# The-Learning-And-Vision-Atelier-LAVA/BUFFER

Measured on AMD Instinct MI355X. Metric: registration pairs/sec, higher is better.
Workload: dtype f32

## Files before the change

### buffer_amd/csrc/convnet_wg.hip

```cpp
#include "common.h"
#include <type_traits>

#define WG_CS 160
#define WG_ROW 22
#define WG_ZERO 154
#define WG_MAXC 128
#define WG_LAYERS 8
#define WG_THREADS 256
#define WG_BUF (WG_MAXC * WG_CS)
#define WG_KSTEP (16 * WG_CS)
#ifndef WG_PIN_FOLD
#define WG_PIN_FOLD 1
#endif
#define WG_BLOCKS 16
#ifdef WG_EXP_NOBAR
#define WG_SYNC() __builtin_amdgcn_sched_barrier(0)
#else
#define WG_SYNC() __syncthreads()
#endif

typedef float wgf4 __attribute__((ext_vector_type(4)));
typedef float wgf2 __attribute__((ext_vector_type(2)));
typedef const __attribute__((address_space(3))) wgf2* wg_lds_f2;

struct CylWgParams {
    const float* wt[WG_LAYERS];
    const float* bias[WG_LAYERS];
    int cin[WG_LAYERS], cout[WG_LAYERS], relu[WG_LAYERS];
    const int* only_if;
#ifdef WG_STAMP
    long long* stamps;
#endif
};
#ifdef WG_STAMP
__device__ long long* wg_stamp_ptr;
#define WG_STAMP_IN(SLOT) if ((threadIdx.x & 63) == 0) wg_stamp_ptr[((size_t)blockIdx.x * 4 + threadIdx.x / 64) * 20 + (SLOT)] = __builtin_amdgcn_s_memtime();
#define WG_STAMP_AT(SLOT) if ((threadIdx.x & 63) == 0) P.stamps[((size_t)blockIdx.x * 4 + w) * 20 + (SLOT)] = __builtin_amdgcn_s_memtime();
#else
#define WG_STAMP_AT(SLOT)
#define WG_STAMP_IN(SLOT)
#endif

__device__ __forceinline__ bool wg_tile(int t, int idx, int& ty, int& tx)
{
    if (t == 0) { const bool a = idx < 10; ty = a ? 0 : 1; tx = a ? idx : idx - 6; return true; }
    if (t == 1) { const bool a = idx < 10, b = idx < 14; ty = a ? 2 : (b ? 1 : 3); tx = a ? idx : (b ? idx - 10 : idx - 6); return true; }
    ty = 3; tx = idx & 7;
    return idx < 8;
}

__device__ __forceinline__ unsigned wg_row_addr(unsigned act_addr, int t, int a, int li, int lk)
{
    int ty, tx;
    const bool ok = wg_tile(t, li, ty, tx);
    const int row = 2 * ty - 1 + a;
    return act_addr + 4u * (unsigned)(lk * WG_CS + ((ok && row >= 0 && row <= 6) ? row * WG_ROW + 2 * tx : WG_ZERO));
}

__device__ __forceinline__ float wg_add(float a, float b) { float r; asm("v_add_f32 %0, %1, %2" : "=v"(r) : "v"(a), "v"(b)); return r; }
__device__ __forceinline__ float wg_sub(float a, float b) { float r; asm("v_sub_f32 %0, %1, %2" : "=v"(r) : "v"(a), "v"(b)); return r; }

__host__ __device__ constexpr int wg_a1(int I) { return I == 0 ? 0 : 1; }
__host__ __device__ constexpr int wg_a2(int I) { return I == 3 ? 3 : 2; }
__host__ __device__ constexpr int wg_te(int I, int T1) { return (I == 3 && T1 == 3) ? 2 : T1; }

__host__ __device__ constexpr bool wg_chains(int I, int T0, int T1)
{
    if (I < 0 || I >= 3) return false;
    const int nt = wg_te(I, T1) - T0, ntn = wg_te(I + 1, T1) - T0;
    return nt >= 1 && ntn >= 1 && (1 / nt) == (1 / ntn) && (1 % nt) == (1 % ntn);
}

#define WG_LOAD2(DST, A0, A1_, OFS)                                                                       \
    {                                                                                                     \
        DST[0] = *(wg_lds_f2)(size_t)((A0) + (OFS));                                                      \
        asm volatile("" : "+v"(A0));                                                                      \
        DST[1] = *(wg_lds_f2)(size_t)((A0) + (OFS) + 8);                                                  \
        asm volatile("" : "+v"(A0));                                                                      \
        DST[2] = *(wg_lds_f2)(size_t)((A1_) + (OFS));                                                     \
        asm volatile("" : "+v"(A1_));                                                                     \
        DST[3] = *(wg_lds_f2)(size_t)((A1_) + (OFS) + 8);                                                 \
        asm volatile("" : "+v"(A1_));                                                                     \
    }

#define WG_LOAD1(DST, A0, OFS)                                                                            \
    {                                                                                                     \
        DST[0] = *(wg_lds_f2)(size_t)((A0) + (OFS));                                                      \
        asm volatile("" : "+v"(A0));                                                                      \
        DST[1] = *(wg_lds_f2)(size_t)((A0) + (OFS) + 8);                                                  \
        asm volatile("" : "+v"(A0));                                                                      \
    }
#define WG_LOAD(BOT_, DST, A0, A1_, OFS)                                                                  \
    {                                                                                                     \
        if constexpr (BOT_) WG_LOAD1(DST, A0, OFS) else WG_LOAD2(DST, A0, A1_, OFS)                       \
    }

typedef unsigned wgu4 __attribute__((ext_vector_type(4)));
__device__ __forceinline__ __amdgpu_buffer_rsrc_t wg_weights(const float* wt)
{
    return __builtin_amdgcn_make_buffer_rsrc((void*)wt, 0, 0x7fffffff, 0x00027000);
}
__device__ __forceinline__ wgf4 wg_ldw(__amdgpu_buffer_rsrc_t rs, unsigned uniform_float_ofs, unsigned lane_byte_ofs)
{
    return __builtin_bit_cast(wgf4, __builtin_amdgcn_raw_buffer_load_b128(rs, lane_byte_ofs, uniform_float_ofs * 4, 0));
}

template <int I, int NN, int T0, int T1, bool PRIMED, int INEXT, bool BOT = false, unsigned KSTEP = WG_KSTEP, bool DIFF = false>
__device__ __forceinline__ void wg_pass(unsigned (&RA)[3][4], __amdgpu_buffer_rsrc_t rs, unsigned wp, unsigned wp_next, unsigned lofs, int niter,
                                        int wstride, wgf4 (&W)[NN][2], wgf4 (&acc)[NN][3][4], wgf2 (&D)[2][4], wgf4 (*Wb)[2] = nullptr, unsigned bofs = 0)
{
    constexpr int A1 = BOT ? I : wg_a1(I), A2 = BOT ? I : wg_a2(I);
    constexpr int TE = BOT ? T1 : wg_te(I, T1);
    constexpr int NT = TE > T0 ? TE - T0 : 1;
    if constexpr (TE <= T0) return;
    constexpr int A1N = BOT ? (INEXT < 0 ? 0 : INEXT) : wg_a1(INEXT < 0 ? 0 : INEXT), A2N = BOT ? A1N : wg_a2(INEXT < 0 ? 0 : INEXT);
    constexpr int NTN = (INEXT < 0 || BOT) ? NT : (wg_te(INEXT, T1) - T0);
    static_assert(INEXT < 0 || (NTN >= 1 && (1 / NT) == (1 / NTN) && (1 % NT) == (1 % NTN)), "steps 0 and 1 of the chained pass have this pass's shape");
    float V[2][4];
    unsigned P[NT][2];
#pragma unroll
    for (int t = 0; t < NT; t++) { P[t][0] = RA[T0 + t][A1]; P[t][1] = RA[T0 + t][A2]; }
    if constexpr (!PRIMED) {
#pragma unroll
        for (int g = 0; g < 2; g++) WG_LOAD(BOT, D[g], P[g % NT][0], P[g % NT][1], (g / NT) * KSTEP)
    }
#define WG_XFORM(BUF)                                                                                     \
    {                                                                                                     \
        float r_[4];                                                                                      \
        _Pragma("unroll") for (int b = 0; b < 4; b++) {                                                   \
            const float da_ = D[BUF][b >> 1][b & 1];                                                      \
            if constexpr (BOT) r_[b] = da_;                                                               \
            else {                                                                                        \
                const float db_ = D[BUF][2 + (b >> 1)][b & 1];                                            \
                r_[b] = I == 1 ? wg_add(da_, db_) : (I == 2 ? wg_sub(db_, da_) : wg_sub(da_, db_));       \
            }                                                                                             \
        }                                                                                                 \
        V[BUF][0] = wg_sub(r_[0], r_[2]); V[BUF][1] = wg_add(r_[1], r_[2]);                               \
        V[BUF][2] = wg_sub(r_[2], r_[1]); V[BUF][3] = wg_sub(r_[1], r_[3]);                               \
    }
    WG_XFORM(0)
#pragma unroll 1
    for (int it = 0; it < niter; it++) {
        const bool more = it + 1 < niter;
        const unsigned wcur = wp + 4 * it * wstride;
        const unsigned wn = more ? wcur + 4 * wstride : wp_next;
        const unsigned adv = more ? 4u * KSTEP : 0u;
        __builtin_amdgcn_sched_barrier(0);
#pragma unroll
        for (int s = 0; s < 4 * NT; s++) {
            const int t = T0 + s % NT, kk = s / NT, g = s + 2;
            if (g < 4 * NT) WG_LOAD(BOT, D[s & 1], P[g % NT][0], P[g % NT][1], (g / NT) * KSTEP)
            else {
                const int t2 = (g - 4 * NT) % NT;
                if ((g - 4 * NT) / NT == 0) { P[t2][0] += adv; P[t2][1] += adv; }
                if constexpr (INEXT >= 0) {
                    unsigned q0 = more ? P[t2][0] : RA[T0 + t2][A1N], q1 = more ? P[t2][1] : RA[T0 + t2][A2N];
                    WG_LOAD(BOT, D[s & 1], q0, q1, ((g - 4 * NT) / NT) * KSTEP)
                } else
                    WG_LOAD(BOT, D[s & 1], P[t2][0], P[t2][1], ((g - 4 * NT) / NT) * KSTEP)
            }
            __builtin_amdgcn_sched_barrier(0);
            if constexpr (DIFF) {
                wgf4 wd[NN];
#pragma unroll
                for (int n = 0; n < NN; n++)
#pragma unroll
                    for (int j = 0; j < 4; j++) wd[n][j] = wg_sub(W[n][kk & 1][j], Wb[n][kk & 1][j]);
                __builtin_amdgcn_sched_barrier(0);
#pragma unroll
                for (int n = 0; n < NN; n++)
#pragma unroll
                    for (int j = 0; j < 4; j++)
                        acc[n][t][j] = __builtin_amdgcn_mfma_f32_16x16x4f32(wd[n][j], V[s & 1][j], acc[n][t][j], 0, 0, 0);
            } else {
#pragma unroll
                for (int n = 0; n < NN; n++)
#pragma unroll
                    for (int j = 0; j < 4; j++)
                        acc[n][t][j] = __builtin_amdgcn_mfma_f32_16x16x4f32(W[n][kk & 1][j], V[s & 1][j], acc[n][t][j], 0, 0, 0);
            }
            __builtin_amdgcn_sched_barrier(0);
            WG_XFORM((s + 1) & 1)
            if (s % NT == NT - 1) {
#pragma unroll
                for (int n = 0; n < NN; n++)
                    W[n][kk & 1] = kk < 2 ? wg_ldw(rs, wcur + n * 256 + (kk + 2) * wstride, lofs) : wg_ldw(rs, wn + n * 256 + (kk - 2) * wstride, lofs);
                if constexpr (DIFF) {
#pragma unroll
                    for (int n = 0; n < NN; n++)
                        Wb[n][kk & 1] = kk < 2 ? wg_ldw(rs, wcur + bofs + n * 256 + (kk + 2) * wstride, lofs) : wg_ldw(rs, wn + bofs + n * 256 + (kk - 2) * wstride, lofs);
                }
            }
            __builtin_amdgcn_sched_barrier(0);
        }
#pragma unroll
        for (int t = 2; t < NT; t++) { P[t][0] += adv; P[t][1] += adv; }
    }
#undef WG_XFORM
}

template <int NN, int T0, int T1, unsigned KSTEP = WG_KSTEP, bool FENCE = false>
__device__ __forceinline__ void wg_round(unsigned (&RA)[3][4], __amdgpu_buffer_rsrc_t rs, unsigned wp, unsigned wp_after, unsigned lofs, int niter,
                                         int wstride, unsigned pstride, const float* __restrict__ bias_lane, wgf4 (&W)[NN][2], wgf4 (&Y)[NN][3][2][2])
{
    using std::integral_constant;
    wgf2 D[2][4];
    wgf4 bv[NN];
#pragma unroll
    for (int n = 0; n < NN; n++) bv[n] = bias_lane ? *reinterpret_cast<const wgf4*>(bias_lane + n * 16) : (wgf4){ 0.f, 0.f, 0.f, 0.f };
    wgf4 acc[NN][3][4];
    float zero = 0.f;
    asm volatile("" : "+v"(zero));
#pragma unroll
    for (int n = 0; n < NN; n++)
#pragma unroll
        for (int t = T0; t < T1; t++)
#pragma unroll
            for (int j = 0; j < 4; j++) acc[n][t][j] = (wgf4){ zero, zero, zero, zero };
    auto run = [&](auto ic) __attribute__((always_inline)) {
        constexpr int I = decltype(ic)::value;
        constexpr int INEXT = (I == 3 || (I == 2 && wg_te(3, T1) <= T0)) ? 0 : I + 1;
        if constexpr (I == 1) {
#pragma unroll
            for (int n = 0; n < NN; n++)
#pragma unroll
                for (int t = T0; t < T1; t++) acc[n][t][1] += bv[n];
        }
        constexpr int ICHAIN = (INEXT != 0 && wg_chains(I, T0, T1)) ? INEXT : -1;
        wg_pass<I, NN, T0, T1, wg_chains(I - 1, T0, T1), ICHAIN, false, KSTEP>(RA, rs, wp + I * pstride, INEXT == 0 ? wp_after : wp + (I + 1) * pstride, lofs, niter, wstride, W, acc, D);
        if constexpr (FENCE) __builtin_amdgcn_sched_barrier(0);
#pragma unroll
        for (int n = 0; n < NN; n++)
#pragma unroll
            for (int t = T0; t < T1; t++) {
                if (I == 3 && t == 2) continue;
                if (I == 2 ? false : t == 2) continue;
                const wgf4 f0 = acc[n][t][0] + acc[n][t][1] + acc[n][t][2];
                const wgf4 f1 = acc[n][t][1] - acc[n][t][2] - acc[n][t][3];
                if constexpr (I == 0) { Y[n][t][1][0] = f0; Y[n][t][1][1] = f1; }
                else if constexpr (I == 1) {
#pragma unroll
                    for (int r = 0; r < 4; r++) {
                        Y[n][t][1][0][r] = __builtin_fmaf(2.f, f0[r], -Y[n][t][1][0][r]);
                        Y[n][t][1][1][r] = __builtin_fmaf(2.f, f1[r], -Y[n][t][1][1][r]);
                    }
                }
                else if constexpr (I == 2) { Y[n][t][0][0] = f0; Y[n][t][0][1] = f1; }
                else { Y[n][t][1][0] -= f0; Y[n][t][1][1] -= f1; }
                if constexpr (FENCE || WG_PIN_FOLD) {
                    if constexpr (I == 2) asm volatile("" : "+v"(Y[n][t][0][0]), "+v"(Y[n][t][0][1]));
                    else asm volatile("" : "+v"(Y[n][t][1][0]), "+v"(Y[n][t][1][1]));
                }
            }
    };
    run(integral_constant<int, 0>{});
    run(integral_constant<int, 1>{});
    run(integral_constant<int, 2>{});
    run(integral_constant<int, 3>{});
}

template <int NN>
__device__ __forceinline__ void wg_round_bottom(unsigned (&RA)[3][4], __amdgpu_buffer_rsrc_t rs, unsigned wp, unsigned wp_after, unsigned lofs, int niter,
                                                int wstride, unsigned pstride, const float* __restrict__ bias_lane, wgf4 (&W)[NN][2], wgf4 (&Y)[NN][3][2][2])
{
    wgf2 D[2][4];
    wgf4 acc[NN][3][4];
    float zero = 0.f;
    asm volatile("" : "+v"(zero));
#pragma unroll
    for (int n = 0; n < NN; n++)
#pragma unroll
        for (int j = 0; j < 4; j++)
            acc[n][2][j] = (j == 1 && bias_lane) ? *reinterpret_cast<const wgf4*>(bias_lane + n * 16) : (wgf4){ zero, zero, zero, zero };
    wgf4 Wb[NN][2];
#pragma unroll
    for (int n = 0; n < NN; n++)
#pragma unroll
        for (int k = 0; k < 2; k++) Wb[n][k] = wg_ldw(rs, wp + 2 * pstride + n * 256 + k * wstride, lofs);
    wg_pass<0, NN, 2, 3, false, 1, true>(RA, rs, wp, wp + pstride, lofs, niter, wstride, W, acc, D);
    wg_pass<1, NN, 2, 3, true, -1, true, WG_KSTEP, true>(RA, rs, wp + pstride, wp_after, lofs, niter, wstride, W, acc, D, Wb, pstride);
#pragma unroll
    for (int n = 0; n < NN; n++) {
        Y[n][2][0][0] = acc[n][2][0] + acc[n][2][1] + acc[n][2][2];
        Y[n][2][0][1] = acc[n][2][1] - acc[n][2][2] - acc[n][2][3];
    }
}

template <bool GLB, int NU = 2>
__device__ __forceinline__ void wg_store_tile(const wgf4 (&Yt)[2][2], int t, int nt, int relu, float* __restrict__ act, float* __restrict__ out_glb,
                                              int li, int lk)
{
    const int n0 = nt * 16 + lk * 4;
    const float lo = relu ? 0.f : -__builtin_inff();
    {
        int ty, tx;
        const bool valid = wg_tile(t, li, ty, tx);
#pragma unroll
        for (int u = 0; u < NU; u++) {
            const int row = 2 * ty + u;
            const bool ok = valid && row < 7;
            if constexpr (GLB) {
                if (ok) {
#pragma unroll
                    for (int r = 0; r < 4; r++) {
                        const float v0 = fmaxf(Yt[u][0][r], lo), v1 = fmaxf(Yt[u][1][r], lo);
                        *reinterpret_cast<wgf2*>(out_glb + (size_t)(n0 + r) * 140 + row * 20 + 2 * tx) = (wgf2){ v0, v1 };
                    }
                }
            } else {
                const int pos = ok ? row * WG_ROW + 2 * tx + 1 : WG_ZERO + 4;
                const int h0 = (ok && tx == 0) ? row * WG_ROW + 21 : WG_ZERO + 4;
                const int h1 = (ok && tx == 9) ? row * WG_ROW : WG_ZERO + 5;
                float* p = act + n0 * WG_CS;
#pragma unroll
                for (int r = 0; r < 4; r++) {
                    const float v0 = fmaxf(Yt[u][0][r], lo), v1 = fmaxf(Yt[u][1][r], lo);
                    p[r * WG_CS + pos] = v0; p[r * WG_CS + pos + 1] = v1;
                    p[r * WG_CS + h0] = v0; p[r * WG_CS + h1] = v1;
                }
            }
        }
    }
}

template <int T0, int T1, bool GLB>
__device__ __forceinline__ void wg_store(const wgf4 (&Y)[3][2][2], int nt, int relu, float* __restrict__ act, float* __restrict__ out_glb,
                                         int li, int lk)
{
#pragma unroll
    for (int t = T0; t < T1; t++) {
        if (t == 2) wg_store_tile<GLB, 1>(Y[t], t, nt, relu, act, out_glb, li, lk);
        else wg_store_tile<GLB, 2>(Y[t], t, nt, relu, act, out_glb, li, lk);
    }
}

__device__ __forceinline__ void wg_addresses(const float* act, int k0, int li, int lk, unsigned (&RA)[3][4])
{
    const unsigned act_addr = (unsigned)(size_t)(__attribute__((address_space(3))) const float*)act + (unsigned)k0 * WG_KSTEP;
#pragma unroll
    for (int t = 0; t < 3; t++)
#pragma unroll
        for (int a = 0; a < 4; a++) RA[t][a] = wg_row_addr(act_addr, t, a, li, lk);
}

#ifndef WG_ADDR_PARK
#define WG_ADDR_PARK 1
#endif
struct WgAddrPark { float a[3][4]; };
__device__ __forceinline__ void wg_park_addresses(const float* act, int li, int lk, WgAddrPark& pk)
{
    const unsigned act_addr = (unsigned)(size_t)(__attribute__((address_space(3))) const float*)act;
#pragma unroll
    for (int t = 0; t < 3; t++)
#pragma unroll
        for (int a = 0; a < 4; a++) {
            const unsigned v = wg_row_addr(act_addr, t, a, li, lk);
            asm volatile("v_accvgpr_write_b32 %0, %1" : "=a"(pk.a[t][a]) : "v"(v));
        }
}
__device__ __forceinline__ unsigned wg_parked(const WgAddrPark& pk, int t, int a)
{
    unsigned v;
    asm volatile("v_accvgpr_read_b32 %0, %1" : "=v"(v) : "a"(pk.a[t][a]));
    return v;
}

template <int NN, int K0, int K1, int KN>
__device__ __forceinline__ void wg_first_weights(__amdgpu_buffer_rsrc_t rs, unsigned wp, unsigned lofs, int wstride, wgf4 (&W)[NN][KN])
{
#pragma unroll
    for (int n = 0; n < NN; n++)
#pragma unroll
        for (int k = K0; k < K1; k++) W[n][k] = wg_ldw(rs, wp + n * 256 + k * wstride, lofs);
}

#define WG_XCH_C 64
template <bool GLB>
__device__ __forceinline__ void wg_layer_ksplit(float* __restrict__ act, float* __restrict__ out_glb, const float* __restrict__ wt,
                                                const float* __restrict__ bias, int cin, int cout, int relu, int w, const WgAddrPark& pk)
{
    int lane = threadIdx.x & (WAVE - 1);
    asm volatile("" : "+v"(lane));
    const int li = lane & 15, lk = lane >> 4;
    const int nt = w & 1, half = w >> 1;
    const int k4 = cin >> 2, kn = k4 >> 1, k0 = half * kn, wstride = 256;
    unsigned RA[3][4];
#if WG_ADDR_PARK
#pragma unroll
    for (int t = 0; t < 3; t++)
#pragma unroll
        for (int a = 0; a < 4; a++) RA[t][a] = wg_parked(pk, t, a) + (unsigned)k0 * WG_KSTEP;
#else
    wg_addresses(act, k0, li, lk, RA);
#endif
    const __amdgpu_buffer_rsrc_t rs = wg_weights(wt);
    const unsigned wp = (unsigned)nt * (WG_BLOCKS * cin * 16) + (unsigned)k0 * wstride;
    const unsigned lofs = lane * 16;
    wgf4 W[1][2];
    wg_first_weights<1, 0, 2>(rs, wp, lofs, wstride, W);
    wgf4 Y[1][3][2][2];
    wg_round<1, 0, 2>(RA, rs, wp, wp, lofs, kn >> 2, wstride, (unsigned)(k4 * wstride), half ? nullptr : bias + nt * 16 + lk * 4, W, Y);
    wg_round_bottom<1>(RA, rs, wp, wp, lofs, kn >> 2, wstride, (unsigned)(k4 * wstride), half ? nullptr : bias + nt * 16 + lk * 4, W, Y);
    wgf4* slot = reinterpret_cast<wgf4*>(act + WG_XCH_C * WG_CS) + nt * 640 + lane;
    if (half) {
#pragma unroll
        for (int q = 0; q < 10; q++) slot[q * 64] = Y[0][q >> 2][(q >> 1) & 1][q & 1];
    }
    WG_STAMP_IN(18)
    WG_SYNC();
    WG_STAMP_IN(19)
    if (!half) {
#pragma unroll
        for (int q = 0; q < 10; q++) Y[0][q >> 2][(q >> 1) & 1][q & 1] += slot[q * 64];
        wg_store<0, 3, GLB>(Y[0], nt, relu, act, out_glb, li, lk);
    }
}

template <bool GLB>
__device__ __forceinline__ void wg_layer_mksplit(float* __restrict__ act, float* __restrict__ out_glb, const float* __restrict__ wt,
                                                 const float* __restrict__ bias, int cin, int cout, int relu, int w, const WgAddrPark& pk)
{
    int lane = threadIdx.x & (WAVE - 1);
    asm volatile("" : "+v"(lane));
    const int li = lane & 15, lk = lane >> 4;
    const int h = w & 1, half = w >> 1;
    const int k4 = cin >> 2, kn = k4 >> 1, k0 = half * kn, wstride = 512;
    unsigned RA[3][4];
#if WG_ADDR_PARK
#pragma unroll
    for (int a = 0; a < 4; a++) {
        const unsigned r0 = wg_parked(pk, 0, a), r1 = wg_parked(pk, 1, a);
        RA[0][a] = (h ? r1 : r0) + (unsigned)k0 * WG_KSTEP; RA[1][a] = RA[0][a]; RA[2][a] = wg_parked(pk, 2, a) + (unsigned)k0 * WG_KSTEP;
    }
#else
    {
        const unsigned act_addr = (unsigned)(size_t)(__attribute__((address_space(3))) const float*)act + (unsigned)k0 * WG_KSTEP;
#pragma unroll
        for (int a = 0; a < 4; a++) { RA[0][a] = wg_row_addr(act_addr, h, a, li, lk); RA[1][a] = RA[0][a]; RA[2][a] = wg_row_addr(act_addr, 2, a, li, lk); }
    }
#endif
    const __amdgpu_buffer_rsrc_t rs = wg_weights(wt);
    const unsigned wp = (unsigned)k0 * wstride;
    const unsigned wpb = wp + (unsigned)h * 256;
    const unsigned lofs = lane * 16;
    const unsigned pstride = (unsigned)(k4 * wstride);
    wgf4 Y[2][3][2][2];
    wgf4 W2[2][2];
    wg_first_weights<2, 0, 2>(rs, wp, lofs, wstride, W2);
    wg_round<2, 0, 1>(RA, rs, wp, wpb, lofs, kn >> 2, wstride, pstride, half ? nullptr : bias + lk * 4, W2, Y);
    wgf4 W1[1][2] = { { W2[0][0], W2[0][1] } };
    wgf4 Yb[1][3][2][2];
    wg_round_bottom<1>(RA, rs, wpb, wpb, lofs, kn >> 2, wstride, pstride, half ? nullptr : bias + h * 16 + lk * 4, W1, Yb);
    wgf4* slot = reinterpret_cast<wgf4*>(act + WG_XCH_C * WG_CS) + h * 640 + lane;
    if (half) {
#pragma unroll
        for (int q = 0; q < 8; q++) slot[q * 64] = Y[q >> 2][0][(q >> 1) & 1][q & 1];
        slot[8 * 64] = Yb[0][2][0][0]; slot[9 * 64] = Yb[0][2][0][1];
    }
    WG_SYNC();
    if (!half) {
#pragma unroll
        for (int q = 0; q < 8; q++) Y[q >> 2][0][(q >> 1) & 1][q & 1] += slot[q * 64];
        Yb[0][2][0][0] += slot[8 * 64]; Yb[0][2][0][1] += slot[9 * 64];
        wg_store_tile<GLB, 2>(Y[0][0], h, 0, relu, act, out_glb, li, lk);
        wg_store_tile<GLB, 2>(Y[1][0], h, 1, relu, act, out_glb, li, lk);
        wg_store_tile<GLB, 1>(Yb[0][2], 2, h, relu, act, out_glb, li, lk);
    }
}

__device__ __forceinline__ void wg_layer_msplit(float* __restrict__ act, const float* __restrict__ wt, const float* __restrict__ bias,
                                                int cin, int cout, int relu, int w, const WgAddrPark& pk)
{
    int lane = threadIdx.x & (WAVE - 1);
    asm volatile("" : "+v"(lane));
    const int li = lane & 15, lk = lane >> 4;
    const int pair = w & 1, h = w >> 1;
    const int k4 = cin >> 2, wstride = 512;
    unsigned RA[3][4];
#if WG_ADDR_PARK
#pragma unroll
    for (int a = 0; a < 4; a++) {
        const unsigned r0 = wg_parked(pk, 0, a), r1 = wg_parked(pk, 1, a);
        RA[0][a] = h ? r1 : r0; RA[1][a] = RA[0][a]; RA[2][a] = wg_parked(pk, 2, a);
    }
#else
    {
        const unsigned act_addr = (unsigned)(size_t)(__attribute__((address_space(3))) const float*)act;
#pragma unroll
        for (int a = 0; a < 4; a++) { RA[0][a] = wg_row_addr(act_addr, h, a, li, lk); RA[1][a] = RA[0][a]; RA[2][a] = wg_row_addr(act_addr, 2, a, li, lk); }
    }
#endif
    const __amdgpu_buffer_rsrc_t rs = wg_weights(wt);
    const unsigned wp = (unsigned)pair * (WG_BLOCKS * cin * 32);
    const unsigned wpb = wp + (unsigned)h * 256;
    const unsigned lofs = lane * 16;
    const unsigned pstride = (unsigned)(k4 * wstride);
    wgf4 Y[2][3][2][2];
    wgf4 W2[2][2];
    wg_first_weights<2, 0, 2>(rs, wp, lofs, wstride, W2);
    wg_round<2, 0, 1>(RA, rs, wp, wpb, lofs, k4 >> 2, wstride, pstride, bias + (2 * pair) * 16 + lk * 4, W2, Y);
    wgf4 W1[1][2] = { { W2[0][0], W2[0][1] } };
    wgf4 Yb[1][3][2][2];
    wg_round_bottom<1>(RA, rs, wpb, wpb, lofs, k4 >> 2, wstride, pstride, bias + (2 * pair + h) * 16 + lk * 4, W1, Yb);
    WG_SYNC();
    wg_store_tile<false, 2>(Y[0][0], h, 2 * pair, relu, act, nullptr, li, lk);
    wg_store_tile<false, 2>(Y[1][0], h, 2 * pair + 1, relu, act, nullptr, li, lk);
    wg_store_tile<false, 1>(Yb[0][2], 2, 2 * pair + h, relu, act, nullptr, li, lk);
}

#ifndef WG_PAIR_NT2
#define WG_PAIR_NT2 1
#endif
#ifndef WG_KSPLIT_PAIRS
#define WG_KSPLIT_PAIRS 1
#endif
__host__ __device__ constexpr int wg_group(int cin, int cout) { return (cout >= 64 || WG_KSPLIT_PAIRS) ? 2 : 1; }

template <int T>
__device__ __forceinline__ void wg_park(const wgf4 (&Y)[2][3][2][2], float (&park)[2][3][16])
{
#pragma unroll
    for (int n = 0; n < 2; n++)
#pragma unroll
        for (int q = 0; q < (T == 2 ? 8 : 16); q++)
            asm volatile("v_accvgpr_write_b32 %0, %1" : "=a"(park[n][T][q]) : "v"(Y[n][T][q >> 3][(q >> 2) & 1][q & 3]));
}

__device__ __forceinline__ void wg_layer_pair(float* __restrict__ act, const float* __restrict__ wt, const float* __restrict__ bias,
                                              int cin, int cout, int relu, int pair, const WgAddrPark& pk)
{
    int lane = threadIdx.x & (WAVE - 1);
    asm volatile("" : "+v"(lane));
    const int li = lane & 15, lk = lane >> 4;
#ifdef WG_EXP_SAMEW_PAIR
    const int k4 = cin >> 2, wstride = relu >> 4;
#else
    const int k4 = cin >> 2, wstride = 512;
#endif
    unsigned RA[3][4];
#if WG_ADDR_PARK
    (void)li;
#pragma unroll
    for (int t = 0; t < 3; t++)
#pragma unroll
        for (int a = 0; a < 4; a++) RA[t][a] = wg_parked(pk, t, a);
#else
    wg_addresses(act, 0, li, lk, RA);
#endif
    const __amdgpu_buffer_rsrc_t rs = wg_weights(wt);
    const unsigned wp = (unsigned)pair * (WG_BLOCKS * cin * 32);
    const unsigned lofs = lane * 16;
    const unsigned pstride = (unsigned)(k4 * wstride);
    wgf4 Y[2][3][2][2];
    const float* bv = bias + (2 * pair) * 16 + lk * 4;
    wgf4 W1[2][2];
    wg_first_weights<2, 0, 2>(rs, wp, lofs, wstride, W1);
    float park[2][3][16];
#if WG_PAIR_NT2
    wg_round<2, 0, 2>(RA, rs, wp, wp, lofs, k4 >> 2, wstride, pstride, bv, W1, Y);
    wg_park<0>(Y, park);
    wg_park<1>(Y, park);
#else
    wg_round<2, 0, 1>(RA, rs, wp, wp, lofs, k4 >> 2, wstride, pstride, bv, W1, Y);
    wg_park<0>(Y, park);
    wg_round<2, 1, 2>(RA, rs, wp, wp, lofs, k4 >> 2, wstride, pstride, bv, W1, Y);
    wg_park<1>(Y, park);
#endif
    wg_round_bottom<2>(RA, rs, wp, wp, lofs, k4 >> 2, wstride, pstride, bv, W1, Y);
    wg_park<2>(Y, park);
    WG_SYNC();
    int lane_s = threadIdx.x & (WAVE - 1);
    asm volatile("" : "+v"(lane_s));
#pragma unroll
    for (int n = 0; n < 2; n++) {
#pragma unroll
        for (int t = 0; t < 3; t++)
#pragma unroll
            for (int q = 0; q < (t == 2 ? 8 : 16); q++)
                asm volatile("v_accvgpr_read_b32 %0, %1" : "=v"(Y[n][t][q >> 3][(q >> 2) & 1][q & 3]) : "a"(park[n][t][q]));
        wg_store<0, 3, false>(Y[n], 2 * pair + n, relu, act, nullptr, lane_s & 15, lane_s >> 4);
    }
}

__device__ __forceinline__ void cyl_net_wg_body(const float* __restrict__ x, const CylWgParams& P, float* __restrict__ y, float* __restrict__ lds)
{
    float* act = lds;
    const int patch = blockIdx.x;
    const int w = __builtin_amdgcn_readfirstlane(threadIdx.x / WAVE);
    WG_STAMP_AT(17)
#ifdef WG_STAMP
    if (threadIdx.x == 0) { P.stamps[(size_t)gridDim.x * 80 + blockIdx.x * 4 + 0] = __builtin_amdgcn_s_memtime(); P.stamps[(size_t)gridDim.x * 80 + blockIdx.x * 4 + 1] = __builtin_amdgcn_s_memrealtime(); }
#endif
    {
        const wgf4* src = reinterpret_cast<const wgf4*>(x + (size_t)patch * P.cin[0] * 140);
        const int nq = P.cin[0] * 35;
        wgf4 v[8];
#pragma unroll
        for (int k = 0; k < 8; k++) {
            const int i = threadIdx.x + k * WG_THREADS;
            if (i < nq) v[k] = __builtin_nontemporal_load(src + i);
        }
        auto put = [&](int i, wgf4 u) __attribute__((always_inline)) {
            const int c = i / 35, q = i - c * 35;
            const int row = q / 5, col = (q - row * 5) * 4;
            float* p = act + c * WG_CS + row * WG_ROW + col + 1;
            p[0] = u[0]; p[1] = u[1]; p[2] = u[2]; p[3] = u[3];
            if (col == 0) p[20] = u[0];
            if (col == 16) p[-17] = u[3];
        };
#pragma unroll
        for (int k = 0; k < 8; k++) {
// ... 138 lines not shown
    BUF_CHECK_HIP(hipMalloc(&P.stamps, (size_t)npatch * (4 * 20 + 4) * sizeof(long long)));
    BUF_CHECK_HIP(hipMemcpyToSymbol(HIP_SYMBOL(wg_stamp_ptr), &P.stamps, sizeof(P.stamps)));
#endif
    if (only_if) k_cyl_net_wg_rerun<<<npatch, WG_THREADS, lds, (hipStream_t)stream>>>(x, P, y);
    else k_cyl_net_wg<<<npatch, WG_THREADS, lds, (hipStream_t)stream>>>(x, P, y);
    if (timed) timing_end((hipStream_t)stream, &span);
    BUF_LAUNCH_CHECK();
#ifdef WG_STAMP
    {
        BUF_CHECK_HIP(hipStreamSynchronize((hipStream_t)stream));
        long long* h = (long long*)malloc((size_t)npatch * (4 * 20 + 4) * sizeof(long long));
        BUF_CHECK_HIP(hipMemcpy(h, P.stamps, (size_t)npatch * (4 * 20 + 4) * sizeof(long long), hipMemcpyDeviceToHost));
        double comp[WG_LAYERS][4] = {}, wait[WG_LAYERS][4] = {}, tot = 0, pre = 0; long n = 0;
        for (int b = npatch / 2; b < npatch; b++, n++)
            for (int w = 0; w < 4; w++) {
                const long long* q = h + ((size_t)b * 4 + w) * 20;
                for (int l = 0; l < WG_LAYERS; l++) { comp[l][w] += (double)(q[2 * l + 1] - q[2 * l]); wait[l][w] += (double)(q[2 * l + 2] - q[2 * l + 1]); }
                if (w == 0) { tot += (double)(q[2 * WG_LAYERS] - q[0]); pre += (double)(q[0] - q[17]); }
            }
        if (n && npatch >= 1024) {
            double dc = 0, dr = 0;
            for (int b = npatch / 2; b < npatch; b++) { const long long* q = h + (size_t)npatch * 80 + (size_t)b * 4; dc += (double)(q[2] - q[0]); dr += (double)(q[3] - q[1]); }
            fprintf(stderr, "  WG_STAMP in-kernel clock: %.0f shader cycles per workgroup over %.0f ticks of the 100 MHz counter -> %.3f GHz\n", dc / n, dr / n, dc / dr * 0.1);
            double c7[4] = {}, b7[4] = {}, s7[4] = {};
            for (int b = npatch / 2; b < npatch; b++)
                for (int w = 0; w < 4; w++) {
                    const long long* q = h + ((size_t)b * 4 + w) * 20;
                    c7[w] += (double)(q[18] - q[14]); b7[w] += (double)(q[19] - q[18]); s7[w] += (double)(q[15] - q[19]);
                }
            fprintf(stderr, "  last layer per wave: K loops %6.0f %6.0f %6.0f %6.0f | barrier %5.0f %5.0f %5.0f %5.0f | add + store %5.0f %5.0f %5.0f %5.0f\n",
                    c7[0] / n, c7[1] / n, c7[2] / n, c7[3] / n, b7[0] / n, b7[1] / n, b7[2] / n, b7[3] / n, s7[0] / n, s7[1] / n, s7[2] / n, s7[3] / n);
            fprintf(stderr, "WG_STAMP: %ld workgroups, layers total %.0f cycles per patch, input phase %.0f\n", n, tot / n, pre / n);
            for (int l = 0; l < WG_LAYERS; l++) {
                const double mf = 40.0 * (P.cin[l] / 4) * (P.cout[l] / 16) / 4;
                fprintf(stderr, "  layer %d %3d->%3d: MFMAs/wave %5.0f | to barrier %7.0f %7.0f %7.0f %7.0f | wait %6.0f %6.0f %6.0f %6.0f | cycles per MFMA slot %.1f\n",
                        l, P.cin[l], P.cout[l], mf, comp[l][0] / n, comp[l][1] / n, comp[l][2] / n, comp[l][3] / n, wait[l][0] / n, wait[l][1] / n,
                        wait[l][2] / n, wait[l][3] / n, (comp[l][0] + wait[l][0]) / n / (2 * mf));
            }
        }
        free(h); (void)hipFree(P.stamps);
    }
#endif
    return BUF_OK;
}
```

Measured before the change: 150.0.

## Compute bottom output row with direct convolution instead of Winograd tile

Replaces the Winograd-based bottom M-tile (row 6) with a direct 2x3 tap convolution that builds combined tap weights in registers and issues 6 MFMAs per k-step per output block. This drops the half-wasted Winograd transform on the single leftover row, cuts its parked accumulators and exchange slots, and removes the BOT/DIFF template paths. In exchange it loads three weight blocks per step and does extra VALU subtracts to form the taps, which could raise register pressure and global load traffic.

```diff
diff --git a/buffer_amd/csrc/convnet_wg.hip b/buffer_amd/csrc/convnet_wg.hip
--- a/buffer_amd/csrc/convnet_wg.hip
+++ b/buffer_amd/csrc/convnet_wg.hip
@@ -45,12 +45,13 @@
 {
     if (t == 0) { const bool a = idx < 10; ty = a ? 0 : 1; tx = a ? idx : idx - 6; return true; }
     if (t == 1) { const bool a = idx < 10, b = idx < 14; ty = a ? 2 : (b ? 1 : 3); tx = a ? idx : (b ? idx - 10 : idx - 6); return true; }
-    ty = 3; tx = idx & 7;
-    return idx < 8;
+    ty = 3; tx = 0;
+    return false;
 }
 
 __device__ __forceinline__ unsigned wg_row_addr(unsigned act_addr, int t, int a, int li, int lk)
 {
+    if (t == 2) return act_addr + 4u * (unsigned)(lk * WG_CS + (a < 2 ? (5 + a) * WG_ROW + li : WG_ZERO));
     int ty, tx;
     const bool ok = wg_tile(t, li, ty, tx);
     const int row = 2 * ty - 1 + a;
@@ -62,14 +63,8 @@
 
 __host__ __device__ constexpr int wg_a1(int I) { return I == 0 ? 0 : 1; }
 __host__ __device__ constexpr int wg_a2(int I) { return I == 3 ? 3 : 2; }
-__host__ __device__ constexpr int wg_te(int I, int T1) { return (I == 3 && T1 == 3) ? 2 : T1; }
-
-__host__ __device__ constexpr bool wg_chains(int I, int T0, int T1)
-{
-    if (I < 0 || I >= 3) return false;
-    const int nt = wg_te(I, T1) - T0, ntn = wg_te(I + 1, T1) - T0;
-    return nt >= 1 && ntn >= 1 && (1 / nt) == (1 / ntn) && (1 % nt) == (1 % ntn);
-}
+
+__host__ __device__ constexpr bool wg_chains(int I) { return I >= 0 && I < 3; }
 
 #define WG_LOAD2(DST, A0, A1_, OFS)                                                                       \
     {                                                                                                     \
@@ -83,17 +78,6 @@
         asm volatile("" : "+v"(A1_));                                                                     \
     }
 
-#define WG_LOAD1(DST, A0, OFS)                                                                            \
-    {                                                                                                     \
-        DST[0] = *(wg_lds_f2)(size_t)((A0) + (OFS));                                                      \
-        asm volatile("" : "+v"(A0));                                                                      \
-        DST[1] = *(wg_lds_f2)(size_t)((A0) + (OFS) + 8);                                                  \
-        asm volatile("" : "+v"(A0));                                                                      \
-    }
-#define WG_LOAD(BOT_, DST, A0, A1_, OFS)                                                                  \
-    {                                                                                                     \
-        if constexpr (BOT_) WG_LOAD1(DST, A0, OFS) else WG_LOAD2(DST, A0, A1_, OFS)                       \
-    }
 
 typedef unsigned wgu4 __attribute__((ext_vector_type(4)));
 __device__ __forceinline__ __amdgpu_buffer_rsrc_t wg_weights(const float* wt)
@@ -105,35 +89,29 @@
     return __builtin_bit_cast(wgf4, __builtin_amdgcn_raw_buffer_load_b128(rs, lane_byte_ofs, uniform_float_ofs * 4, 0));
 }
 
-template <int I, int NN, int T0, int T1, bool PRIMED, int INEXT, bool BOT = false, unsigned KSTEP = WG_KSTEP, bool DIFF = false>
+template <int I, int NN, int T0, int T1, bool PRIMED, int INEXT, unsigned KSTEP = WG_KSTEP>
 __device__ __forceinline__ void wg_pass(unsigned (&RA)[3][4], __amdgpu_buffer_rsrc_t rs, unsigned wp, unsigned wp_next, unsigned lofs, int niter,
-                                        int wstride, wgf4 (&W)[NN][2], wgf4 (&acc)[NN][3][4], wgf2 (&D)[2][4], wgf4 (*Wb)[2] = nullptr, unsigned bofs = 0)
-{
-    constexpr int A1 = BOT ? I : wg_a1(I), A2 = BOT ? I : wg_a2(I);
-    constexpr int TE = BOT ? T1 : wg_te(I, T1);
-    constexpr int NT = TE > T0 ? TE - T0 : 1;
-    if constexpr (TE <= T0) return;
-    constexpr int A1N = BOT ? (INEXT < 0 ? 0 : INEXT) : wg_a1(INEXT < 0 ? 0 : INEXT), A2N = BOT ? A1N : wg_a2(INEXT < 0 ? 0 : INEXT);
-    constexpr int NTN = (INEXT < 0 || BOT) ? NT : (wg_te(INEXT, T1) - T0);
-    static_assert(INEXT < 0 || (NTN >= 1 && (1 / NT) == (1 / NTN) && (1 % NT) == (1 % NTN)), "steps 0 and 1 of the chained pass have this pass's shape");
+                                        int wstride, wgf4 (&W)[NN][2], wgf4 (&acc)[NN][3][4], wgf2 (&D)[2][4])
+{
+    static_assert(T0 < T1 && T1 <= 2, "the Winograd M-tiles (M-tile 2 is wg_round_direct's)");
+    constexpr int A1 = wg_a1(I), A2 = wg_a2(I);
+    constexpr int NT = T1 - T0;
+    constexpr int A1N = wg_a1(INEXT < 0 ? 0 : INEXT), A2N = wg_a2(INEXT < 0 ? 0 : INEXT);
     float V[2][4];
     unsigned P[NT][2];
 #pragma unroll
     for (int t = 0; t < NT; t++) { P[t][0] = RA[T0 + t][A1]; P[t][1] = RA[T0 + t][A2]; }
     if constexpr (!PRIMED) {
 #pragma unroll
-        for (int g = 0; g < 2; g++) WG_LOAD(BOT, D[g], P[g % NT][0], P[g % NT][1], (g / NT) * KSTEP)
+        for (int g = 0; g < 2; g++) WG_LOAD2(D[g], P[g % NT][0], P[g % NT][1], (g / NT) * KSTEP)
     }
 #define WG_XFORM(BUF)                                                                                     \
     {                                                                                                     \
         float r_[4];                                                                                      \
         _Pragma("unroll") for (int b = 0; b < 4; b++) {                                                   \
             const float da_ = D[BUF][b >> 1][b & 1];                                                      \
-            if constexpr (BOT) r_[b] = da_;                                                               \
-            else {                                                                                        \
-                const float db_ = D[BUF][2 + (b >> 1)][b & 1];                                            \
-                r_[b] = I == 1 ? wg_add(da_, db_) : (I == 2 ? wg_sub(db_, da_) : wg_sub(da_, db_));       \
-            }                                                                                             \
+            const float db_ = D[BUF][2 + (b >> 1)][b & 1];                                                \
+            r_[b] = I == 1 ? wg_add(da_, db_) : (I == 2 ? wg_sub(db_, da_) : wg_sub(da_, db_));           \
         }                                                                                                 \
         V[BUF][0] = wg_sub(r_[0], r_[2]); V[BUF][1] = wg_add(r_[1], r_[2]);                               \
         V[BUF][2] = wg_sub(r_[2], r_[1]); V[BUF][3] = wg_sub(r_[1], r_[3]);                               \
@@ -149,47 +127,28 @@
 #pragma unroll
         for (int s = 0; s < 4 * NT; s++) {
             const int t = T0 + s % NT, kk = s / NT, g = s + 2;
-            if (g < 4 * NT) WG_LOAD(BOT, D[s & 1], P[g % NT][0], P[g % NT][1], (g / NT) * KSTEP)
+            if (g < 4 * NT) WG_LOAD2(D[s & 1], P[g % NT][0], P[g % NT][1], (g / NT) * KSTEP)
             else {
                 const int t2 = (g - 4 * NT) % NT;
                 if ((g - 4 * NT) / NT == 0) { P[t2][0] += adv; P[t2][1] += adv; }
                 if constexpr (INEXT >= 0) {
                     unsigned q0 = more ? P[t2][0] : RA[T0 + t2][A1N], q1 = more ? P[t2][1] : RA[T0 + t2][A2N];
-                    WG_LOAD(BOT, D[s & 1], q0, q1, ((g - 4 * NT) / NT) * KSTEP)
+                    WG_LOAD2(D[s & 1], q0, q1, ((g - 4 * NT) / NT) * KSTEP)
                 } else
-                    WG_LOAD(BOT, D[s & 1], P[t2][0], P[t2][1], ((g - 4 * NT) / NT) * KSTEP)
+                    WG_LOAD2(D[s & 1], P[t2][0], P[t2][1], ((g - 4 * NT) / NT) * KSTEP)
             }
             __builtin_amdgcn_sched_barrier(0);
-            if constexpr (DIFF) {
-                wgf4 wd[NN];
-#pragma unroll
-                for (int n = 0; n < NN; n++)
-#pragma unroll
-                    for (int j = 0; j < 4; j++) wd[n][j] = wg_sub(W[n][kk & 1][j], Wb[n][kk & 1][j]);
-                __builtin_amdgcn_sched_barrier(0);
-#pragma unroll
-                for (int n = 0; n < NN; n++)
-#pragma unroll
-                    for (int j = 0; j < 4; j++)
-                        acc[n][t][j] = __builtin_amdgcn_mfma_f32_16x16x4f32(wd[n][j], V[s & 1][j], acc[n][t][j], 0, 0, 0);
-            } else {
-#pragma unroll
-                for (int n = 0; n < NN; n++)
-#pragma unroll
-                    for (int j = 0; j < 4; j++)
-                        acc[n][t][j] = __builtin_amdgcn_mfma_f32_16x16x4f32(W[n][kk & 1][j], V[s & 1][j], acc[n][t][j], 0, 0, 0);
-            }
+#pragma unroll
+            for (int n = 0; n < NN; n++)
+#pragma unroll
+                for (int j = 0; j < 4; j++)
+                    acc[n][t][j] = __builtin_amdgcn_mfma_f32_16x16x4f32(W[n][kk & 1][j], V[s & 1][j], acc[n][t][j], 0, 0, 0);
             __builtin_amdgcn_sched_barrier(0);
             WG_XFORM((s + 1) & 1)
             if (s % NT == NT - 1) {
 #pragma unroll
                 for (int n = 0; n < NN; n++)
                     W[n][kk & 1] = kk < 2 ? wg_ldw(rs, wcur + n * 256 + (kk + 2) * wstride, lofs) : wg_ldw(rs, wn + n * 256 + (kk - 2) * wstride, lofs);
-                if constexpr (DIFF) {
-#pragma unroll
-                    for (int n = 0; n < NN; n++)
-                        Wb[n][kk & 1] = kk < 2 ? wg_ldw(rs, wcur + bofs + n * 256 + (kk + 2) * wstride, lofs) : wg_ldw(rs, wn + bofs + n * 256 + (kk - 2) * wstride, lofs);
-                }
             }
             __builtin_amdgcn_sched_barrier(0);
         }
@@ -219,22 +178,20 @@
             for (int j = 0; j < 4; j++) acc[n][t][j] = (wgf4){ zero, zero, zero, zero };
     auto run = [&](auto ic) __attribute__((always_inline)) {
         constexpr int I = decltype(ic)::value;
-        constexpr int INEXT = (I == 3 || (I == 2 && wg_te(3, T1) <= T0)) ? 0 : I + 1;
+        constexpr int INEXT = I == 3 ? 0 : I + 1;
         if constexpr (I == 1) {
 #pragma unroll
             for (int n = 0; n < NN; n++)
 #pragma unroll
                 for (int t = T0; t < T1; t++) acc[n][t][1] += bv[n];
         }
-        constexpr int ICHAIN = (INEXT != 0 && wg_chains(I, T0, T1)) ? INEXT : -1;
-        wg_pass<I, NN, T0, T1, wg_chains(I - 1, T0, T1), ICHAIN, false, KSTEP>(RA, rs, wp + I * pstride, INEXT == 0 ? wp_after : wp + (I + 1) * pstride, lofs, niter, wstride, W, acc, D);
+        constexpr int ICHAIN = (INEXT != 0 && wg_chains(I)) ? INEXT : -1;
+        wg_pass<I, NN, T0, T1, wg_chains(I - 1), ICHAIN, KSTEP>(RA, rs, wp + I * pstride, INEXT == 0 ? wp_after : wp + (I + 1) * pstride, lofs, niter, wstride, W, acc, D);
         if constexpr (FENCE) __builtin_amdgcn_sched_barrier(0);
 #pragma unroll
         for (int n = 0; n < NN; n++)
 #pragma unroll
             for (int t = T0; t < T1; t++) {
-                if (I == 3 && t == 2) continue;
-                if (I == 2 ? false : t == 2) continue;
                 const wgf4 f0 = acc[n][t][0] + acc[n][t][1] + acc[n][t][2];
                 const wgf4 f1 = acc[n][t][1] - acc[n][t][2] - acc[n][t][3];
                 if constexpr (I == 0) { Y[n][t][1][0] = f0; Y[n][t][1][1] = f1; }
@@ -259,34 +216,87 @@
     run(integral_constant<int, 3>{});
 }
 
+typedef const __attribute__((address_space(3))) float* wg_lds_f1;
+#define WG_LOADD(DST, A0, OFS)                                                                            \
+    {                                                                                                     \
+        _Pragma("unroll") for (int a_ = 0; a_ < 2; a_++)                                                  \
+            _Pragma("unroll") for (int b_ = 0; b_ < 3; b_++)                                              \
+                DST[a_ * 3 + b_] = *(wg_lds_f1)(size_t)((A0) + (OFS) + 4 * (a_ * WG_ROW + b_));           \
+    }
 template <int NN>
-__device__ __forceinline__ void wg_round_bottom(unsigned (&RA)[3][4], __amdgpu_buffer_rsrc_t rs, unsigned wp, unsigned wp_after, unsigned lofs, int niter,
-                                                int wstride, unsigned pstride, const float* __restrict__ bias_lane, wgf4 (&W)[NN][2], wgf4 (&Y)[NN][3][2][2])
-{
-    wgf2 D[2][4];
-    wgf4 acc[NN][3][4];
+__device__ __forceinline__ void wg_round_direct(unsigned row5, __amdgpu_buffer_rsrc_t rs, unsigned wp, unsigned lofs, int niter, int wstride,
+                                                unsigned pstride, const float* __restrict__ bias_lane, wgf4 (&W)[NN][2], wgf4 (&Y)[NN])
+{
+    wgf4 Wr[3][NN][2];
+#pragma unroll
+    for (int n = 0; n < NN; n++)
+#pragma unroll
+        for (int k = 0; k < 2; k++) {
+            Wr[0][n][k] = W[n][k];
+            Wr[1][n][k] = wg_ldw(rs, wp + pstride + n * 256 + k * wstride, lofs);
+            Wr[2][n][k] = wg_ldw(rs, wp + 2 * pstride + n * 256 + k * wstride, lofs);
+        }
+    float X[2][6];
+    unsigned pa = row5;
+    WG_LOADD(X[0], pa, 0)
+    WG_LOADD(X[1], pa, WG_KSTEP)
+    wgf4 acc[NN][2];
     float zero = 0.f;
     asm volatile("" : "+v"(zero));
 #pragma unroll
-    for (int n = 0; n < NN; n++)
-#pragma unroll
-        for (int j = 0; j < 4; j++)
-            acc[n][2][j] = (j == 1 && bias_lane) ? *reinterpret_cast<const wgf4*>(bias_lane + n * 16) : (wgf4){ zero, zero, zero, zero };
-    wgf4 Wb[NN][2];
-#pragma unroll
-    for (int n = 0; n < NN; n++)
-#pragma unroll
-        for (int k = 0; k < 2; k++) Wb[n][k] = wg_ldw(rs, wp + 2 * pstride + n * 256 + k * wstride, lofs);
-    wg_pass<0, NN, 2, 3, false, 1, true>(RA, rs, wp, wp + pstride, lofs, niter, wstride, W, acc, D);
-    wg_pass<1, NN, 2, 3, true, -1, true, WG_KSTEP, true>(RA, rs, wp + pstride, wp_after, lofs, niter, wstride, W, acc, D, Wb, pstride);
-#pragma unroll
     for (int n = 0; n < NN; n++) {
-        Y[n][2][0][0] = acc[n][2][0] + acc[n][2][1] + acc[n][2][2];
-        Y[n][2][0][1] = acc[n][2][1] - acc[n][2][2] - acc[n][2][3];
-    }
-}
-
-template <bool GLB, int NU = 2>
+        acc[n][0] = bias_lane ? *reinterpret_cast<const wgf4*>(bias_lane + n * 16) : (wgf4){ zero, zero, zero, zero };
+        acc[n][1] = (wgf4){ zero, zero, zero, zero };
+    }
+    float G[NN][6];
+#define WG_TAPS(SLOT)                                                                                     \
+    _Pragma("unroll") for (int n = 0; n < NN; n++) {                                                      \
+        const wgf4 u0_ = Wr[0][n][SLOT], u1_ = Wr[1][n][SLOT], u2_ = Wr[2][n][SLOT];                      \
+        const float d1_ = wg_sub(u1_[1], u2_[1]), d2_ = wg_sub(u1_[2], u2_[2]);                           \
+        G[n][0] = u0_[0]; G[n][1] = wg_sub(u0_[1], u0_[2]); G[n][2] = u0_[3];                             \
+        G[n][3] = wg_sub(u1_[0], u2_[0]); G[n][4] = wg_sub(d1_, d2_); G[n][5] = wg_sub(u1_[3], u2_[3]);   \
+    }
+#define WG_RELOAD(SLOT, OFS)                                                                              \
+    _Pragma("unroll") for (int n = 0; n < NN; n++)                                                        \
+        _Pragma("unroll") for (int blk = 0; blk < 3; blk++) Wr[blk][n][SLOT] = wg_ldw(rs, (OFS) + blk * pstride + n * 256, lofs);
+    WG_TAPS(0)
+    WG_RELOAD(0, wp + 2 * wstride)
+#pragma unroll 1
+    for (int it = 0; it < niter; it++) {
+        const bool more = it + 1 < niter;
+        const unsigned wcur = wp + 4 * it * wstride;
+        const unsigned wn = more ? wcur + 4 * wstride : wp;
+        const unsigned adv = more ? 4u * WG_KSTEP : 0u;
+        __builtin_amdgcn_sched_barrier(0);
+#pragma unroll
+        for (int s = 0; s < 4; s++) {
+#pragma unroll
+            for (int b = 0; b < 3; b++)
+#pragma unroll
+                for (int a = 0; a < 2; a++)
+#pragma unroll
+                    for (int n = 0; n < NN; n++)
+                        acc[n][a] = __builtin_amdgcn_mfma_f32_16x16x4f32(G[n][a * 3 + b], X[s & 1][a * 3 + b], acc[n][a], 0, 0, 0);
+            __builtin_amdgcn_sched_barrier(0);
+            if (s < 2) WG_LOADD(X[s & 1], pa, (s + 2) * WG_KSTEP)
+            else {
+                if (s == 2) pa += adv;
+                WG_LOADD(X[s & 1], pa, (s - 2) * WG_KSTEP)
+            }
+            __builtin_amdgcn_sched_barrier(0);
+            WG_TAPS((s + 1) & 1)
+            if (s == 0) WG_RELOAD(1, wcur + 3 * wstride)
+            else WG_RELOAD((s + 1) & 1, wn + (s - 1) * wstride)
+            __builtin_amdgcn_sched_barrier(0);
+        }
+    }
+#undef WG_TAPS
+#undef WG_RELOAD
+#pragma unroll
+    for (int n = 0; n < NN; n++) Y[n] = acc[n][0] + acc[n][1];
+}
+
+template <bool GLB>
 __device__ __forceinline__ void wg_store_tile(const wgf4 (&Yt)[2][2], int t, int nt, int relu, float* __restrict__ act, float* __restrict__ out_glb,
                                               int li, int lk)
 {
@@ -296,7 +306,7 @@
         int ty, tx;
         const bool valid = wg_tile(t, li, ty, tx);
 #pragma unroll
-        for (int u = 0; u < NU; u++) {
+        for (int u = 0; u < 2; u++) {
             const int row = 2 * ty + u;
             const bool ok = valid && row < 7;
             if constexpr (GLB) {
@@ -323,14 +333,34 @@
     }
 }
 
+template <bool GLB>
+__device__ __forceinline__ void wg_store_row6(const wgf4& Yr, int nt, int relu, float* __restrict__ act, float* __restrict__ out_glb, int li, int lk)
+{
+    const int n0 = nt * 16 + lk * 4;
+    const float lo = relu ? 0.f : -__builtin_inff();
+    if constexpr (GLB) {
+#pragma unroll
+        for (int r = 0; r < 4; r++) out_glb[(size_t)(n0 + r) * 140 + 6 * 20 + li] = fmaxf(Yr[r], lo);
+    } else {
+        const int pos = 6 * WG_ROW + li + 1;
+        const int h0 = li == 0 ? 6 * WG_ROW + 21 : WG_ZERO + 4;
+        float* p = act + n0 * WG_CS;
+#pragma unroll
+        for (int r = 0; r < 4; r++) {
+            const float v = fmaxf(Yr[r], lo);
+            p[r * WG_CS + pos] = v; p[r * WG_CS + h0] = v;
+        }
+    }
+}
+
 template <int T0, int T1, bool GLB>
 __device__ __forceinline__ void wg_store(const wgf4 (&Y)[3][2][2], int nt, int relu, float* __restrict__ act, float* __restrict__ out_glb,
                                          int li, int lk)
 {
 #pragma unroll
     for (int t = T0; t < T1; t++) {
-        if (t == 2) wg_store_tile<GLB, 1>(Y[t], t, nt, relu, act, out_glb, li, lk);
-        else wg_store_tile<GLB, 2>(Y[t], t, nt, relu, act, out_glb, li, lk);
+        if (t == 2) wg_store_row6<GLB>(Y[t][0][0], nt, relu, act, out_glb, li, lk);
+        else wg_store_tile<GLB>(Y[t], t, nt, relu, act, out_glb, li, lk);
     }
 }
 
@@ -340,7 +370,7 @@
 #pragma unroll
     for (int t = 0; t < 3; t++)
 #pragma unroll
-        for (int a = 0; a < 4; a++) RA[t][a] = wg_row_addr(act_addr, t, a, li, lk);
+        for (int a = 0; a < (t == 2 ? 1 : 4); a++) RA[t][a] = wg_row_addr(act_addr, t, a, li, lk);
 }
 
 #ifndef WG_ADDR_PARK
@@ -353,7 +383,7 @@
 #pragma unroll
     for (int t = 0; t < 3; t++)
 #pragma unroll
-        for (int a = 0; a < 4; a++) {
+        for (int a = 0; a < (t == 2 ? 1 : 4); a++) {
             const unsigned v = wg_row_addr(act_addr, t, a, li, lk);
             asm volatile("v_accvgpr_write_b32 %0, %1" : "=a"(pk.a[t][a]) : "v"(v));
         }
@@ -389,7 +419,7 @@
 #pragma unroll
     for (int t = 0; t < 3; t++)
 #pragma unroll
-        for (int a = 0; a < 4; a++) RA[t][a] = wg_parked(pk, t, a) + (unsigned)k0 * WG_KSTEP;
+        for (int a = 0; a < (t == 2 ? 1 : 4); a++) RA[t][a] = wg_parked(pk, t, a) + (unsigned)k0 * WG_KSTEP;
 #else
     wg_addresses(act, k0, li, lk, RA);
 #endif
@@ -400,18 +430,20 @@
     wg_first_weights<1, 0, 2>(rs, wp, lofs, wstride, W);
     wgf4 Y[1][3][2][2];
     wg_round<1, 0, 2>(RA, rs, wp, wp, lofs, kn >> 2, wstride, (unsigned)(k4 * wstride), half ? nullptr : bias + nt * 16 + lk * 4, W, Y);
-    wg_round_bottom<1>(RA, rs, wp, wp, lofs, kn >> 2, wstride, (unsigned)(k4 * wstride), half ? nullptr : bias + nt * 16 + lk * 4, W, Y);
+    wgf4 Yb[1];
+    wg_round_direct<1>(RA[2][0], rs, wp, lofs, kn >> 2, wstride, (unsigned)(k4 * wstride), half ? nullptr : bias + nt * 16 + lk * 4, W, Yb);
+    Y[0][2][0][0] = Yb[0];
     wgf4* slot = reinterpret_cast<wgf4*>(act + WG_XCH_C * WG_CS) + nt * 640 + lane;
     if (half) {
 #pragma unroll
-        for (int q = 0; q < 10; q++) slot[q * 64] = Y[0][q >> 2][(q >> 1) & 1][q & 1];
+        for (int q = 0; q < 9; q++) slot[q * 64] = Y[0][q >> 2][(q >> 1) & 1][q & 1];
     }
     WG_STAMP_IN(18)
     WG_SYNC();
     WG_STAMP_IN(19)
     if (!half) {
 #pragma unroll
-        for (int q = 0; q < 10; q++) Y[0][q >> 2][(q >> 1) & 1][q & 1] += slot[q * 64];
+        for (int q = 0; q < 9; q++) Y[0][q >> 2][(q >> 1) & 1][q & 1] += slot[q * 64];
         wg_store<0, 3, GLB>(Y[0], nt, relu, act, out_glb, li, lk);
     }
 }
@@ -430,13 +462,15 @@
 #pragma unroll
     for (int a = 0; a < 4; a++) {
         const unsigned r0 = wg_parked(pk, 0, a), r1 = wg_parked(pk, 1, a);
-        RA[0][a] = (h ? r1 : r0) + (unsigned)k0 * WG_KSTEP; RA[1][a] = RA[0][a]; RA[2][a] = wg_parked(pk, 2, a) + (unsigned)k0 * WG_KSTEP;
-    }
+        RA[0][a] = (h ? r1 : r0) + (unsigned)k0 * WG_KSTEP; RA[1][a] = RA[0][a];
+    }
+    RA[2][0] = wg_parked(pk, 2, 0) + (unsigned)k0 * WG_KSTEP;
 #else
     {
         const unsigned act_addr = (unsigned)(size_t)(__attribute__((address_space(3))) const float*)act + (unsigned)k0 * WG_KSTEP;
 #pragma unroll
-        for (int a = 0; a < 4; a++) { RA[0][a] = wg_row_addr(act_addr, h, a, li, lk); RA[1][a] = RA[0][a]; RA[2][a] = wg_row_addr(act_addr, 2, a, li, lk); }
+        for (int a = 0; a < 4; a++) { RA[0][a] = wg_row_addr(act_addr, h, a, li, lk); RA[1][a] = RA[0][a]; }
+        RA[2][0] = wg_row_addr(act_addr, 2, 0, li, lk);
     }
 #endif
     const __amdgpu_buffer_rsrc_t rs = wg_weights(wt);
@@ -449,22 +483,22 @@
     wg_first_weights<2, 0, 2>(rs, wp, lofs, wstride, W2);
     wg_round<2, 0, 1>(RA, rs, wp, wpb, lofs, kn >> 2, wstride, pstride, half ? nullptr : bias + lk * 4, W2, Y);
     wgf4 W1[1][2] = { { W2[0][0], W2[0][1] } };
-    wgf4 Yb[1][3][2][2];
-    wg_round_bottom<1>(RA, rs, wpb, wpb, lofs, kn >> 2, wstride, pstride, half ? nullptr : bias + h * 16 + lk * 4, W1, Yb);
+    wgf4 Yb[1];
+    wg_round_direct<1>(RA[2][0], rs, wpb, lofs, kn >> 2, wstride, pstride, half ? nullptr : bias + h * 16 + lk * 4, W1, Yb);
     wgf4* slot = reinterpret_cast<wgf4*>(act + WG_XCH_C * WG_CS) + h * 640 + lane;
     if (half) {
 #pragma unroll
         for (int q = 0; q < 8; q++) slot[q * 64] = Y[q >> 2][0][(q >> 1) & 1][q & 1];
-        slot[8 * 64] = Yb[0][2][0][0]; slot[9 * 64] = Yb[0][2][0][1];
+        slot[8 * 64] = Yb[0];
     }
     WG_SYNC();
     if (!half) {
 #pragma unroll
         for (int q = 0; q < 8; q++) Y[q >> 2][0][(q >> 1) & 1][q & 1] += slot[q * 64];
-        Yb[0][2][0][0] += slot[8 * 64]; Yb[0][2][0][1] += slot[9 * 64];
-        wg_store_tile<GLB, 2>(Y[0][0], h, 0, relu, act, out_glb, li, lk);
-        wg_store_tile<GLB, 2>(Y[1][0], h, 1, relu, act, out_glb, li, lk);
-        wg_store_tile<GLB, 1>(Yb[0][2], 2, h, relu, act, out_glb, li, lk);
+        Yb[0] += slot[8 * 64];
+        wg_store_tile<GLB>(Y[0][0], h, 0, relu, act, out_glb, li, lk);
+        wg_store_tile<GLB>(Y[1][0], h, 1, relu, act, out_glb, li, lk);
+        wg_store_row6<GLB>(Yb[0], h, relu, act, out_glb, li, lk);
     }
 }
 
@@ -481,13 +515,15 @@
 #pragma unroll
     for (int a = 0; a < 4; a++) {
         const unsigned r0 = wg_parked(pk, 0, a), r1 = wg_parked(pk, 1, a);
-        RA[0][a] = h ? r1 : r0; RA[1][a] = RA[0][a]; RA[2][a] = wg_parked(pk, 2, a);
-    }
+        RA[0][a] = h ? r1 : r0; RA[1][a] = RA[0][a];
+    }
+    RA[2][0] = wg_parked(pk, 2, 0);
 #else
     {
         const unsigned act_addr = (unsigned)(size_t)(__attribute__((address_space(3))) const float*)act;
 #pragma unroll
-        for (int a = 0; a < 4; a++) { RA[0][a] = wg_row_addr(act_addr, h, a, li, lk); RA[1][a] = RA[0][a]; RA[2][a] = wg_row_addr(act_addr, 2, a, li, lk); }
+        for (int a = 0; a < 4; a++) { RA[0][a] = wg_row_addr(act_addr, h, a, li, lk); RA[1][a] = RA[0][a]; }
+        RA[2][0] = wg_row_addr(act_addr, 2, 0, li, lk);
     }
 #endif
     const __amdgpu_buffer_rsrc_t rs = wg_weights(wt);
@@ -500,12 +536,12 @@
     wg_first_weights<2, 0, 2>(rs, wp, lofs, wstride, W2);
     wg_round<2, 0, 1>(RA, rs, wp, wpb, lofs, k4 >> 2, wstride, pstride, bias + (2 * pair) * 16 + lk * 4, W2, Y);
     wgf4 W1[1][2] = { { W2[0][0], W2[0][1] } };
-    wgf4 Yb[1][3][2][2];
-    wg_round_bottom<1>(RA, rs, wpb, wpb, lofs, k4 >> 2, wstride, pstride, bias + (2 * pair + h) * 16 + lk * 4, W1, Yb);
+    wgf4 Yb[1];
+    wg_round_direct<1>(RA[2][0], rs, wpb, lofs, k4 >> 2, wstride, pstride, bias + (2 * pair + h) * 16 + lk * 4, W1, Yb);
     WG_SYNC();
-    wg_store_tile<false, 2>(Y[0][0], h, 2 * pair, relu, act, nullptr, li, lk);
-    wg_store_tile<false, 2>(Y[1][0], h, 2 * pair + 1, relu, act, nullptr, li, lk);
-    wg_store_tile<false, 1>(Yb[0][2], 2, 2 * pair + h, relu, act, nullptr, li, lk);
+    wg_store_tile<false>(Y[0][0], h, 2 * pair, relu, act, nullptr, li, lk);
+    wg_store_tile<false>(Y[1][0], h, 2 * pair + 1, relu, act, nullptr, li, lk);
+    wg_store_row6<false>(Yb[0], 2 * pair + h, relu, act, nullptr, li, lk);
 }
 
 #ifndef WG_PAIR_NT2
@@ -522,7 +558,7 @@
 #pragma unroll
     for (int n = 0; n < 2; n++)
 #pragma unroll
-        for (int q = 0; q < (T == 2 ? 8 : 16); q++)
+        for (int q = 0; q < (T == 2 ? 4 : 16); q++)
             asm volatile("v_accvgpr_write_b32 %0, %1" : "=a"(park[n][T][q]) : "v"(Y[n][T][q >> 3][(q >> 2) & 1][q & 3]));
 }
 
@@ -543,7 +579,7 @@
 #pragma unroll
     for (int t = 0; t < 3; t++)
 #pragma unroll
-        for (int a = 0; a < 4; a++) RA[t][a] = wg_parked(pk, t, a);
+        for (int a = 0; a < (t == 2 ? 1 : 4); a++) RA[t][a] = wg_parked(pk, t, a);
 #else
     wg_addresses(act, 0, li, lk, RA);
 #endif
@@ -566,7 +602,9 @@
     wg_round<2, 1, 2>(RA, rs, wp, wp, lofs, k4 >> 2, wstride, pstride, bv, W1, Y);
     wg_park<1>(Y, park);
 #endif
-    wg_round_bottom<2>(RA, rs, wp, wp, lofs, k4 >> 2, wstride, pstride, bv, W1, Y);
+    wgf4 Yb[2];
+    wg_round_direct<2>(RA[2][0], rs, wp, lofs, k4 >> 2, wstride, pstride, bv, W1, Yb);
+    Y[0][2][0][0] = Yb[0]; Y[1][2][0][0] = Yb[1];
     wg_park<2>(Y, park);
     WG_SYNC();
     int lane_s = threadIdx.x & (WAVE - 1);
@@ -576,7 +614,7 @@
 #pragma unroll
         for (int t = 0; t < 3; t++)
 #pragma unroll
-            for (int q = 0; q < (t == 2 ? 8 : 16); q++)
+            for (int q = 0; q < (t == 2 ? 4 : 16); q++)
                 asm volatile("v_accvgpr_read_b32 %0, %1" : "=v"(Y[n][t][q >> 3][(q >> 2) & 1][q & 3]) : "a"(park[n][t][q]));
         wg_store<0, 3, false>(Y[n], 2 * pair + n, relu, act, nullptr, lane_s & 15, lane_s >> 4);
     }
@@ -781,7 +819,7 @@
                     c7[0] / n, c7[1] / n, c7[2] / n, c7[3] / n, b7[0] / n, b7[1] / n, b7[2] / n, b7[3] / n, s7[0] / n, s7[1] / n, s7[2] / n, s7[3] / n);
             fprintf(stderr, "WG_STAMP: %ld workgroups, layers total %.0f cycles per patch, input phase %.0f\n", n, tot / n, pre / n);
             for (int l = 0; l < WG_LAYERS; l++) {
-                const double mf = 40.0 * (P.cin[l] / 4) * (P.cout[l] / 16) / 4;
+                const double mf = 38.0 * (P.cin[l] / 4) * (P.cout[l] / 16) / 4;
                 fprintf(stderr, "  layer %d %3d->%3d: MFMAs/wave %5.0f | to barrier %7.0f %7.0f %7.0f %7.0f | wait %6.0f %6.0f %6.0f %6.0f | cycles per MFMA slot %.1f\n",
                         l, P.cin[l], P.cout[l], mf, comp[l][0] / n, comp[l][1] / n, comp[l][2] / n, comp[l][3] / n, wait[l][0] / n, wait[l][1] / n,
                         wait[l][2] / n, wait[l][3] / n, (comp[l][0] + wait[l][0]) / n / (2 * mf));
```

Result: faster. 155.1 (median of 6 runs) (+3.4%).
